# AlanConfluent/flink

Hardware: AMD Instinct MI355X
Metric: records/sec aggregated (1M-key tumbling SUM) (higher is better)
Workload: dtype int64

## Files before the change

flink_amd/_abi.py:

```python
import ctypes as C

import numpy as np

FWA_ABI_VERSION = 5
FWA_MAX_AGGS = 8
FWA_MAX_COLS = 8

TUMBLE, SLIDE, CUMULATE, SESSION = 0, 1, 2, 3
WINDOW_KINDS = {"TUMBLE": TUMBLE, "SLIDE": SLIDE, "HOP": SLIDE, "CUMULATE": CUMULATE, "SESSION": SESSION}
SEM_DATASTREAM, SEM_TABLE = 0, 1
SEMANTICS = {"DATASTREAM": SEM_DATASTREAM, "TABLE": SEM_TABLE}
KEY_JAVA_LONG, KEY_BINROW_BIGINT, KEY_PREHASHED, KEY_GROUP_PREFIXED = 0, 1, 2, 3

AGG_KINDS = {
    "COUNT": 0, "SUM_I64": 1, "SUM_F32": 2, "SUM_F64": 3, "MIN_I64": 4, "MAX_I64": 5,
    "MIN_F32": 6, "MAX_F32": 7, "MIN_F64": 8, "MAX_F64": 9, "AVG_I64": 10, "AVG_F32": 11,
    "AVG_F64": 12, "COUNT_COL": 13,
    "SUM_DEC": 14, "AVG_DEC": 15, "SUM_DEC128": 16, "AVG_DEC128": 17,
    "SUM_I32": 18, "MIN_I32": 19, "MAX_I32": 20, "FIRST_64": 21, "FIRST_32": 22,
    "MINBY_I64": 23, "MAXBY_I64": 24, "MINBY_I32": 25, "MAXBY_I32": 26, "MINBY_F64": 27, "MAXBY_F64": 28,
    "MINBY_F32": 29, "MAXBY_F32": 30, "SEL_64": 31, "SEL_32": 32,
    "COUNT_DISTINCT": 33,
}
AGG_DISTINCT = 0x100
# ... 41 lines not shown
    w = np.frombuffer(memoryview(raw).cast("B"), np.uint64).reshape(-1, 2)
    out = np.empty(w.shape[0], object)
    for i in range(w.shape[0]):
        u = int(w[i, 0]) | (int(w[i, 1]) << 64)
        out[i] = u - (1 << 128) if u >= 1 << 127 else u
    return out

STATUS = {0: "OK", -1: "E_ARG", -2: "E_TS_MIN", -3: "E_KEYGROUP", -4: "E_MERGE_LATE", -5: "E_OOM",
          -6: "E_DEVICE", -7: "E_UNSUPPORTED", -8: "E_STATE", -9: "E_CORRUPT", -10: "E_INTERNAL"}

CFG_DYNAMIC_GAP = 0x1
CFG_LATE_INDICES = 0x2
CFG_RECORD_LISTS = 0x4
CFG_REDUCE = 0x8
CFG_BY_LAST = 0x10
CFG_DISTINCT_RANGE = 0x20
CFG_DISTINCT_SESSION = 0x40
CFG_F32_FOLD = 0x80

PUSH_DEVICE_PTRS = 0x1
PUSH_ASYNC = 0x2

OPT_KEY_TABLE_SHAPE = 34
OPT_HEAP_KEY_POS = 35


def key_table_shape(value):
    return int(value) & 0xff, int(value) >> 8

LONG_MIN = -(1 << 63)
LONG_MAX = (1 << 63) - 1


class AggSpec(C.Structure):
    _fields_ = [("kind", C.c_int32), ("col", C.c_int32)]


class Config(C.Structure):
    _fields_ = [
        ("abi_version", C.c_int32), ("window_kind", C.c_int32), ("semantics", C.c_int32),
        ("key_kind", C.c_int32), ("size_ms", C.c_int64), ("slide_ms", C.c_int64),
        ("offset_ms", C.c_int64), ("gap_ms", C.c_int64), ("allowed_lateness_ms", C.c_int64),
        ("max_parallelism", C.c_int32), ("kg_start", C.c_int32), ("kg_end", C.c_int32),
        ("num_aggs", C.c_int32), ("aggs", AggSpec * FWA_MAX_AGGS), ("device", C.c_int32),
        ("output_on_device", C.c_int32), ("key_capacity", C.c_int64), ("max_batch", C.c_int64),
        ("flags", C.c_int32), ("gap_col", C.c_int32), ("tz_n", C.c_int32), ("nullable_cols", C.c_int32),
# ... 123 lines not shown
```

flink_amd/csrc/engine.hip:

```cpp
#include <hip/hip_runtime.h>
#include <hipcub/device/device_radix_sort.hpp>
#include <hipcub/device/device_scan.hpp>

#include <algorithm>
#include <cstdio>
#include <cstdlib>
#include <cstring>
#include <map>
#include <set>
#include <string>
#include <vector>

#include "../../include/flink_amd.h"
#include "java_math.h"
#include "dec_view.h"

#define LONG_MIN_J ((int64_t)0x8000000000000000LL)
#define LONG_MAX_J ((int64_t)0x7fffffffffffffffLL)

namespace {

#include "ingest.inc"
#include "ingest_launch.inc"

// ... 755 lines not shown
    int32_t slot[kRelTabN];
    uint8_t code[kRelTabN], fresh[kRelTabN];
};

__global__ void push_reset_kernel(DevStatus* st, unsigned long long* want, int32_t nwant, uint32_t* bcnt, int32_t nbcnt,
                                  int32_t* rel2slot, RelTab tab) {
    const int32_t t = blockIdx.x * blockDim.x + threadIdx.x;
    const int32_t nt = gridDim.x * blockDim.x;
    if (rel2slot) {
        uint8_t* code = (uint8_t*)(rel2slot + kRelCap);
        uint8_t* fresh = code + kRelCap;
        for (int32_t i = t; i < kRelCap; i += nt) {
            const int32_t j = i - tab.lo;
            const bool in = j >= 0 && j < tab.n;
            rel2slot[i] = in ? tab.slot[j] : -1;
            code[i] = in ? tab.code[j] : kCodeSlow;
            fresh[i] = in ? tab.fresh[j] : (uint8_t)0;
        }
    }
    if (t == 0) {
        st->error = 0; st->spill_n = 0; st->want_n = 0; st->key_full = 0;
        st->rows = 0;
        st->dropped = 0; st->late_fire = 0; st->max_q = 0; st->min_q = ~0ull; st->ovf_n = 0; st->strag_n = 0; st->wide_n = 0;
    }
    for (int32_t i = t; i < nwant; i += nt) want[i] = 0ull;
    for (int32_t i = t; i < nbcnt; i += nt) bcnt[i] = 0u;
}

struct SlotList { int32_t n, id[15]; };
__global__ void reset_slots_kernel(unsigned long long* const* slot_base, const int32_t* list, SlotList inl, int64_t stride,
                                   int32_t* touched, const EngineConst* __restrict__ cp) {
    const EngineConst& c = *cp;
    const int32_t sid = inl.n ? inl.id[blockIdx.y] : list[blockIdx.y];
    const int32_t slot = sid < 0 ? ~sid : sid;
    if (sid < 0) {
        if (blockIdx.x == 0 && threadIdx.x == 0) touched[slot] = 0;
        return;
    }
    unsigned long long* base = slot_base[slot];
    const int64_t step = (int64_t)gridDim.x * blockDim.x;
    const int64_t m = stride / 2;
    for (int col = 0; col < c.nacc; ++col) {
        const unsigned long long v = (col > 0 && c.acc_kind[col] == ACC_MIN_ORD) ? ~0ull : 0ull;
        ulonglong2* p = (ulonglong2*)(base + (int64_t)col * stride);
        const ulonglong2 v2 = make_ulonglong2(v, v);
        int64_t i = (int64_t)blockIdx.x * blockDim.x + threadIdx.x;
// ... 220 lines not shown
    bool st_ready = false;
    bool af_pend = false;
    bool af_gpu = false;
    int64_t af_rows = 0;
    int64_t* h_af_rows = nullptr;
    hipEvent_t ev_af = nullptr;
    int32_t* h_touched = nullptr;
    int32_t h_touched_cap = 0;
    bool sparse = false;
    bool red = false;
    unsigned long long* d_rk = nullptr;
    int32_t* d_iota = nullptr;
    int64_t iota_cap = 0;
    int64_t iota_n = 0;
    bool iota_pending = false, iota_ran = false;
    int32_t* d_rslots = nullptr;
    int64_t rslots_cap = 0;
    int64_t rk_cap = 0;
    int64_t red_seq_base = 0;
    SpState* sp = nullptr;
    int32_t opt_pre = -1, opt_mp = -1, opt_narrow = -1, opt_cells = -1;
    int32_t opt_variant = 0;
    int64_t stragglers = 0;
    bool rows_zero = false;
    int64_t fused_fires = 0;
    int64_t reset_launches = 0;
    int32_t push_epoch = 0;
    unsigned long long* d_rsum = nullptr;
    bool rs_valid = false;
    int64_t rs_q0 = 0;
    int32_t rs_u0 = 0, rs_epoch = 0;
    int32_t rs_k = 4;
    bool rs_on = true;
    int64_t rs_used = 0;
    int64_t opt_out_min = 0;
    bool opt_partials_v1 = false;
    int32_t opt_profile = 0;
    void* d_mf = nullptr;
    size_t mf_bytes = 0;
    double mf_groups_per_row = 1.0;
    double mf_capx = 2.0;
    int32_t opt_fire_partials = -1;
    int32_t opt_dec_wrap_null = 0;
    int32_t opt_heap_key_pos = -1;
    int64_t mf_calls = 0, mf_fallbacks = 0;
    int64_t* d_dr = nullptr;
// ... 1317 lines not shown
    int64_t qmin = LONG_MAX_J, qmax = LONG_MIN_J;
    bool republish = false;
    std::vector<int32_t> late_idx;
    for (int round = 0;; ++round) {
        if (round == 0 && status_enqueued && e->st_ready) rc = FWA_OK;
        else rc = (round == 0 && status_enqueued) ? wait_status(e) : sync_status(e);
        e->st_ready = false;
        if (rc) return rc;
        if (e->v2_timing_pending) {
            float ms = 0.f;
            HIPCHK(e, hipEventElapsedTime(&ms, e->ev[4], e->ev[5]));
            e->partition_ms += ms;
            e->ingest_ms += ms;
            HIPCHK(e, hipEventElapsedTime(&ms, e->ev[6], e->ev[7]));
            e->combine_ms += ms;
            e->ingest_ms += ms;
            e->v2_timing_pending = false;
        }
        if (!ran_v2 || round > 0) { rc = account_ingest(e); if (rc) return rc; }
        const DevStatus st = *e->h_st;
        if (ran_v2 && round == 0 && (int64_t)st.ovf_n * 64 > n) e->pre = true;
        if (ran_v2 && round == 0 && (int64_t)st.strag_n * 64 > n) e->mp = true;
        if (ran_v2 && round == 0) e->stragglers += st.strag_n;
        if (ran_v2 && round == 0 && e->narrow_used && (int64_t)st.wide_n * 64 > n) e->narrow = false;
        if (round == 0) settle_push_stale(e);
        if (st.error) {
            const char* m = st.error == FWA_E_KEYGROUP ? "Key group is not in the owned KeyGroupRange (StateTable.getMapForKeyGroup)"
                          : st.error == FWA_E_TS_MIN ? "Record has Long.MIN_VALUE timestamp (= no timestamp marker)."
                          : st.error == FWA_E_OOM ? (st.key_full ? "key table full: raise fwa_config.key_capacity" : "slice want-set overflow")
                                                  : "device error";
            return fail(e, st.error, m);
        }
        if (st.late_fire) {
            const size_t o = late_idx.size();
            late_idx.resize(o + st.late_fire);
            HIPCHK(e, hipMemcpy(late_idx.data() + o, e->d_late, 4 * (size_t)st.late_fire, hipMemcpyDeviceToHost));
        }
        dropped += (int64_t)st.dropped;
        if (st.max_q) qmax = std::max<int64_t>(qmax, jm::unord_i64(st.max_q));
        if (st.min_q != ~0ull) qmin = std::min<int64_t>(qmin, jm::unord_i64(st.min_q));
        if (round == 0) e->steady = ran_v2 && st.spill_n == 0;
        if (st.spill_n == 0) break;
        if (round > 64) return fail(e, FWA_E_STATE, "miss replay did not converge");
        std::vector<unsigned long long> want(kWantCap);
        HIPCHK(e, hipMemcpy(want.data(), e->d_want, sizeof(unsigned long long) * kWantCap, hipMemcpyDeviceToHost));
        for (unsigned long long w : want) {
// ... 1337 lines not shown
        case FWA_OPT_HEAP_KEY_POS:
            if (value < 0 || value > (e->dist ? e->dist->ucfg.num_aggs : e->dec ? e->dec->ucfg.num_aggs : e->cfg.num_aggs))
                return fail(e, FWA_E_ARG, "FWA_OPT_HEAP_KEY_POS: the key's tuple position, 0 .. num_aggs");
            e->opt_heap_key_pos = (int32_t)value;
            return FWA_OK;
        case FWA_OPT_DISTINCT_SLOTS:
            if (!e->dist) return fail(e, FWA_E_UNSUPPORTED, "FWA_OPT_DISTINCT_SLOTS: no COUNT(DISTINCT) aggregate");
            if (e->dist->d_tab) return fail(e, FWA_E_STATE, "FWA_OPT_DISTINCT_SLOTS: before the first push");
            if (value < 64 || (value & (value - 1)) || value > ((int64_t)1 << 40))
                return fail(e, FWA_E_ARG, "FWA_OPT_DISTINCT_SLOTS: a power of two >= 64");
            e->dist->first_slots = value;
            return FWA_OK;
        case FWA_OPT_F32_FOLD_SLOTS:
            if (!e->fold) return fail(e, FWA_E_UNSUPPORTED, "FWA_OPT_F32_FOLD_SLOTS: no SUM_F32 aggregate under FWA_CFG_F32_FOLD");
            if (e->fold->d_tab) return fail(e, FWA_E_STATE, "FWA_OPT_F32_FOLD_SLOTS: before the first push");
            if (value < 64 || (value & (value - 1)) || value > ((int64_t)1 << 31))
                return fail(e, FWA_E_ARG, "FWA_OPT_F32_FOLD_SLOTS: a power of two >= 64");
            e->fold->first_slots = value;
            return FWA_OK;
        case FWA_OPT_F32_FOLD_REBUILDS: case FWA_OPT_F32_FOLD_RESOLVE_US: case FWA_OPT_F32_FOLD_SORT_US:
        case FWA_OPT_F32_FOLD_RUNS_US: case FWA_OPT_F32_FOLD_ROWS_US:
        case FWA_OPT_DISTINCT_LIVE: case FWA_OPT_DISTINCT_REBUILDS: case FWA_OPT_STRAGGLERS: case FWA_OPT_KEY_TABLE_DIGEST:
        case FWA_OPT_DISTINCT_INDEX_US: case FWA_OPT_DISTINCT_COUNT_US: case FWA_OPT_DISTINCT_COUNT_STEPS:
        case FWA_OPT_FAST_SLICE_PUSHES: case FWA_OPT_KEY_TABLE_SHAPE:
            return fail(e, FWA_E_ARG, "read-only option");
        default: return fail(e, FWA_E_ARG, "unknown option");
    }
}

int fwa_get_option(const fwa_engine* e, int32_t option, int64_t* value) {
    if (!e || !value) return FWA_E_ARG;
    auto eff = [](int32_t opt, bool adaptive_on) -> int64_t { return opt == 1 || (opt != 0 && adaptive_on) ? 1 : 0; };
    switch (option) {
        case FWA_OPT_SKEW_MERGE: *value = eff(e->opt_pre, e->pre); return FWA_OK;
        case FWA_OPT_WINDOW_PASSES: *value = eff(e->opt_mp, e->mp); return FWA_OK;
        case FWA_OPT_NARROW_ENTRIES: *value = eff(e->opt_narrow, e->narrow); return FWA_OK;
        case FWA_OPT_SESSION_CELLS: *value = eff(e->opt_cells, e->cell_skip <= 0); return FWA_OK;
        case FWA_OPT_OUT_MIN_ROWS: *value = e->opt_out_min > 0 ? e->opt_out_min : ((int64_t)1 << 22); return FWA_OK;
        case FWA_OPT_PARTIALS_ONE_PASS: *value = e->opt_partials_v1 ? 1 : 0; return FWA_OK;
        case FWA_OPT_SP_TABLE: case FWA_OPT_SP_FMAX: case FWA_OPT_SP_BUDGET:
            if (!e->sp) return FWA_E_UNSUPPORTED;
            *value = option == FWA_OPT_SP_TABLE ? e->sp->T : option == FWA_OPT_SP_FMAX ? (e->sp->fmax ? e->sp->fmax : kSpMaxF)
                                                                                    : (int64_t)e->sp->budget;
            return FWA_OK;
        case FWA_OPT_PROFILE: *value = e->opt_profile; return FWA_OK;
        case FWA_OPT_SESSION_PATH: *value = e->sess_path; return FWA_OK;
        case FWA_OPT_INGEST_VARIANT: *value = e->opt_variant; return FWA_OK;
        case FWA_OPT_SLIDE_CARRIED: *value = e->rs_used; return FWA_OK;
        case FWA_OPT_FIRE_PARTIALS: *value = e->mf_calls - e->mf_fallbacks; return FWA_OK;
        case FWA_OPT_DEC_WRAP_NULL: *value = e->opt_dec_wrap_null; return FWA_OK;
        case FWA_OPT_HEAP_KEY_POS: *value = e->opt_heap_key_pos; return FWA_OK;
        case FWA_OPT_FUSED_FIRES: *value = e->fused_fires; return FWA_OK;
        case FWA_OPT_RESET_LAUNCHES: *value = e->reset_launches; return FWA_OK;
        case FWA_OPT_STALE_RETIRES: *value = e->stale_retires; return FWA_OK;
        case FWA_OPT_STRAGGLERS: *value = e->stragglers; return FWA_OK;
        case FWA_OPT_FAST_SLICE_PUSHES: *value = e->fast_slice_pushes; return FWA_OK;
        case FWA_OPT_KEY_TABLE_SHAPE:
            if (e->sparse) return FWA_E_UNSUPPORTED;
            *value = (int64_t)e->seg_log | ((int64_t)e->part_bits << 8);
            return FWA_OK;
        case FWA_OPT_KEY_TABLE_DIGEST: {
            std::vector<unsigned long long> table((size_t)e->capacity + 1);
            if (!e->d_keys || hipStreamSynchronize(e->stream) != hipSuccess ||
                hipMemcpy(table.data(), e->d_keys, 8 * table.size(), hipMemcpyDeviceToHost) != hipSuccess) return FWA_E_DEVICE;
            uint64_t h = 0xcbf29ce484222325ull;
            for (unsigned long long w : table)
                for (int b = 0; b < 8; ++b) h = (h ^ ((w >> (8 * b)) & 0xff)) * 0x100000001b3ull;
            *value = (int64_t)h;
            return FWA_OK;
        }
        case FWA_OPT_DISTINCT_SLOTS: case FWA_OPT_DISTINCT_LIVE: case FWA_OPT_DISTINCT_REBUILDS:
            if (!e->dist) return FWA_E_UNSUPPORTED;
            *value = option == FWA_OPT_DISTINCT_SLOTS ? (e->dist->slots ? e->dist->slots : e->dist->first_slots)
                   : option == FWA_OPT_DISTINCT_LIVE ? e->dist->live : e->dist->rebuilds;
            return FWA_OK;
        case FWA_OPT_F32_FOLD_SLOTS: case FWA_OPT_F32_FOLD_REBUILDS: case FWA_OPT_F32_FOLD_RESOLVE_US:
        case FWA_OPT_F32_FOLD_SORT_US: case FWA_OPT_F32_FOLD_RUNS_US: case FWA_OPT_F32_FOLD_ROWS_US:
            if (!e->fold) return FWA_E_UNSUPPORTED;
// ... 60 lines not shown
```

flink_amd/csrc/ingest.inc:

```

#ifdef FWA_KPROF
#define KPROF(p) ((p) != nullptr)
#else
#define KPROF(p) false
#endif

constexpr int kBlock = 256;
constexpr uint64_t kEmptyKey = 0x8000000000000000ull;
constexpr int kBucket = 8;
constexpr int32_t kWantCap = 1 << 14;


struct DirEntry {
    int64_t q;
    int32_t slot;
    int32_t flags;
    int64_t thr;
    int64_t first_maxts;
};

struct DevStatus {
    int32_t error;
    int32_t spill_n;
    int32_t want_n;
    int32_t key_full;
    unsigned long long dropped;
    unsigned long long n_keys;
    unsigned long long late_fire;
    unsigned long long rows;
    unsigned long long max_q;
    unsigned long long min_q;
    int32_t pad;
    int32_t pad2;
    unsigned long long sess_live;
    unsigned long long drop_n;
    int32_t ovf_n;
    int32_t strag_n;
    int32_t wide_n;
    int32_t pad3;
};

__device__ __forceinline__ void note_drop(int32_t* list, DevStatus* st, bool drop, int64_t i) {
    if (!list) return;
    const unsigned long long m = __ballot(drop);
    if (!m) return;
    const int lane = threadIdx.x & 63;
    const int ld = __ffsll((long long)m) - 1;
    unsigned long long b = 0;
    if (lane == ld) b = atomicAdd(&st->drop_n, (unsigned long long)__popcll(m));
    b = __shfl(b, ld);
    if (drop) list[b + __popcll(m & ((1ull << lane) - 1))] = (int32_t)i;
}

enum AccKind : int32_t { ACC_NONE = 0, ACC_ADD_I64 = 1, ACC_ADD_F64 = 2, ACC_MIN_ORD = 3, ACC_MAX_ORD = 4, ACC_PAYLOAD = 5 };

struct AggDesc {
    int32_t kind;
    int32_t col;
    int32_t acc;
    int32_t acc_kind;
    int32_t vslot;
    int32_t alias;
// ... 718 lines not shown
            atomicMin(&a.st->min_q, (unsigned long long)jm::ord_i64(a.q_base + (int64_t)relmin));
        }
    }
    if (relmin != ~0u)
        for (uint32_t r = relmin + (uint32_t)lane; r <= relmax; r += 64) {
            const int32_t slot = a.rel2slot[r];
            if (slot >= 0 && a.touched[slot] != a.epoch) a.touched[slot] = a.epoch;
        }
}

struct CombineArgs {
    const unsigned long long* b_key;
    const unsigned long long* b_val0;
    const unsigned long long* b_val1;
    const uint16_t* b_rel;
    const uint16_t* b_n;
    const uint32_t* b_cnt;
    int64_t capb;
    int32_t seg_log, np, sl;
    int32_t sub_major;
    const int32_t* rel2slot;
    const uint8_t* relfresh;
    int32_t stale;
    int64_t q_base;
    unsigned long long* key_table;
    unsigned long long* const* slot_base;
    int64_t stride;
    DevStatus* st;
    long long* prof;
};

__device__ __forceinline__ unsigned long long ident_of(int acc_kind) { return acc_kind == ACC_MIN_ORD ? ~0ull : 0ull; }

__device__ __forceinline__ unsigned long long carried_ord(unsigned long long raw, int kind) {
    switch (kind) {
        case FWA_MIN_I64: case FWA_MAX_I64: case FWA_MINBY_I64: case FWA_MAXBY_I64: return jm::ord_i64((int64_t)raw);
        case FWA_MIN_I32: case FWA_MAX_I32: return jm::ord_i64((int64_t)(int32_t)(uint32_t)raw);
        case FWA_MIN_F32: case FWA_MAX_F32:
            return jm::ord_bits64((uint64_t)__double_as_longlong((double)__uint_as_float((uint32_t)raw)));
        default: return jm::ord_bits64(raw);
    }
}

__device__ __forceinline__ double carried_f64(unsigned long long raw, int kind) {
    return (kind == FWA_SUM_F32 || kind == FWA_AVG_F32) ? (double)__uint_as_float((uint32_t)raw)
                                                         : __longlong_as_double((long long)raw);
// ... 67 lines not shown
            stale_range(a, s_lo_, s_hi_); \
            for (int r_ = max(s_lo_, lo + SL); r_ <= s_hi_; ++r_) if (a.relfresh[r_] == 2) ident_seg(r_); \
        } } while (0)
#define STALE_SIDE(NACC) do { \
        int s_lo_, s_hi_; \
        stale_range(a, s_lo_, s_hi_); \
        if (p == a.np - 1) stale_side<TH>(a, s_lo_, s_hi_, tid, NACC, kind_of); } while (0)

constexpr int kStragL = 256;
struct StragL {
    uint32_t g, n;
    int32_t rel, pad;
    unsigned long long x0, x1;
};

__device__ __forceinline__ uint32_t kswz(uint32_t s) { return s ^ (((s >> 5) & 3u) << 1); }


typedef __attribute__((address_space(1))) unsigned long long g_u64;
typedef const __attribute__((address_space(1))) unsigned long long* gc_u64_ptr;

constexpr int32_t kLeanEmpty = (int32_t)0x80000000;
constexpr int32_t kLeanForeign = (int32_t)0x80000001;
typedef int32_t lean_i4 __attribute__((ext_vector_type(4)));

__device__ __forceinline__ uint32_t kswz32(uint32_t s) { return s ^ (((s >> 6) & 1u) << 2); }

__device__ __forceinline__ int32_t lean_key_image(unsigned long long k) {
    if (k == kEmptyKey) return kLeanEmpty;
    const bool narrow = (int64_t)(int32_t)(uint32_t)k == (int64_t)k && (uint32_t)k - 0x80000000u > 1u;
    return narrow ? (int32_t)(uint32_t)k : kLeanForeign;
}

template <int BT>
__device__ __forceinline__ void lean_pin(const lean_i4* qa, const lean_i4* qb) {
    static_assert(BT >= 1 && BT <= 4, "batch size");
    if constexpr (BT == 1) asm volatile("" : : "v"(qa[0]), "v"(qb[0]));
    else if constexpr (BT == 2) asm volatile("" : : "v"(qa[0]), "v"(qb[0]), "v"(qa[1]), "v"(qb[1]));
    else if constexpr (BT == 3) asm volatile("" : : "v"(qa[0]), "v"(qb[0]), "v"(qa[1]), "v"(qb[1]), "v"(qa[2]), "v"(qb[2]));
    else asm volatile("" : : "v"(qa[0]), "v"(qb[0]), "v"(qa[1]), "v"(qb[1]), "v"(qa[2]), "v"(qb[2]), "v"(qa[3]), "v"(qb[3]));
}

__device__ __forceinline__ int32_t lean_match(const lean_i4& qa, const lean_i4& qb, int32_t kk) {
    int32_t t = -1;
    unsigned long long m0, m1, m2, m3, m4, m5, m6, m7;
    asm("v_cmp_eq_u32_e64 %8, %16, %17\n\t"
// ... 24 lines not shown
    const unsigned long long p = (unsigned long long)xlo * c1l;
    const uint32_t z1lo = (uint32_t)p;
    const uint32_t z1hi = (uint32_t)(p >> 32) + xlo * c1h + (s & (0u - 4u * c1l));
    const uint32_t ylo = z1lo ^ ((z1lo >> 27) | (z1hi << 5));
    const uint32_t yhi = z1hi ^ (z1hi >> 27);
    const unsigned long long q = (unsigned long long)ylo * c2l;
    const uint32_t z2lo = (uint32_t)q;
    const uint32_t z2hi = (uint32_t)(q >> 32) + __umul24(ylo, c2h) + __umul24(yhi, c2l);
    const uint32_t h = z2lo ^ ((z2lo >> 31) | (z2hi << 1));
    return h & smask & ~(uint32_t)(kBucket - 1);
}

template <bool kMax>
__device__ __forceinline__ int lean_wave_red(int v) {
    auto step = [](int x, int y) { return kMax ? max(x, y) : (int)min((uint32_t)x, (uint32_t)y); };
    v = step(v, __builtin_amdgcn_update_dpp(0, v, 0xB1, 0xf, 0xf, true));
    v = step(v, __builtin_amdgcn_update_dpp(0, v, 0x4E, 0xf, 0xf, true));
    v = step(v, __builtin_amdgcn_update_dpp(0, v, 0x141, 0xf, 0xf, true));
    v = step(v, __builtin_amdgcn_update_dpp(0, v, 0x140, 0xf, 0xf, true));
    return step(step(__builtin_amdgcn_readlane(v, 0), __builtin_amdgcn_readlane(v, 16)),
                step(__builtin_amdgcn_readlane(v, 32), __builtin_amdgcn_readlane(v, 48)));
}

template <int IT, int BT, int SL, int TH>
__device__ __forceinline__ void combine3_lean(const CombineArgs& a, const EngineConst& c) {
    extern __shared__ __attribute__((aligned(16))) unsigned char smem[];
    static_assert(IT % BT == 0, "whole batches");
    static_assert(TH / kSub == 64, "one wave per sub-bucket");
    constexpr int kWaves = TH / 64;
    const int tid = threadIdx.x, lane = tid & 63, wv = tid >> 6;
    const int p = blockIdx.x;
    const int seg = 1 << a.seg_log;
    const uint32_t smask = (uint32_t)seg - 1u;
    __shared__ StragL s_strag[kStragL];
    __shared__ int s_sn, s_first;
    int32_t* lkey = (int32_t*)smem;
    uint32_t* lcnt = (uint32_t*)(smem + (size_t)seg * 8);
    unsigned long long* lacc = (unsigned long long*)(smem + (size_t)seg * 8 + (size_t)SL * seg * 4);
    int* s_mm = (int*)(smem + (size_t)seg * 8 + (size_t)SL * seg * 4 + (size_t)SL * seg * 8);
    int* s_new = s_mm + 4 * kWaves;
    long long pt = clock64();
    long long pacc[8] = {0, 0, 0, 0, 0, 0, 0, 0};
#define PMARK(k) do { if (KPROF(a.prof)) { const long long _t = clock64(); pacc[k] += _t - pt; pt = _t; } } while (0)
    unsigned long long* gkeys = a.key_table + ((int64_t)p << a.seg_log);
    for (int i = tid; i < seg; i += TH) lkey[kswz32((uint32_t)i)] = lean_key_image(gkeys[i]);
    for (int i = tid; i < SL * seg; i += TH) { lcnt[i] = 0; lacc[i] = 0ull; }
    if (tid == 0) { *s_new = 0; s_sn = 0; s_first = 0x7fffffff; }
    if (tid < 3) { s_mm[2 * tid] = 0x7fffffff; s_mm[2 * tid + 1] = -1; }
    constexpr int64_t kChunk = (int64_t)IT * 64;
    const int my_cnt = __builtin_amdgcn_readfirstlane((int)min((int64_t)a.b_cnt[p * kSub + wv], a.capb));
    const int64_t boff = (int64_t)bucket_base(p, wv, a.np, a.sub_major) * a.capb;
    int64_t cnt = 0;
    for (int s2 = 0; s2 < kSub; ++s2) cnt = max(cnt, min((int64_t)a.b_cnt[p * kSub + s2], a.capb));
    const gc_u64_ptr bk = (const gc_u64_ptr)(a.b_key + boff);
    const __attribute__((address_space(1))) uint16_t* br = (const __attribute__((address_space(1))) uint16_t*)(a.b_rel + boff);
    int lo = 0x7fffffff;
    auto kind_of = [](int) { return (int)ACC_ADD_I64; };
    auto ident_seg = [&](int r) { stale_ident<TH>(a, r, (int64_t)p << a.seg_log, ((int64_t)p + 1) << a.seg_log, tid, 2, kind_of); };
    STALE_SIDE(2);
    auto flush = [&](int rel) {
        constexpr int kPer = 4096 / TH;
        const int w = rel & (SL - 1);
        const int32_t slot = (rel >= 0 && rel < kRelCap) ? a.rel2slot[rel] : -1;
        g_u64* base = slot >= 0 ? (g_u64*)a.slot_base[slot] : nullptr;
        const int fr = (slot >= 0 && a.relfresh) ? (int)a.relfresh[rel] : 0;
        const bool fresh = fr != 0;
        const bool all = fr == 2;
        uint32_t k[kPer];
        unsigned long long x[kPer];
        int64_t g[kPer];
#pragma unroll
// ... 78 lines not shown
            __syncthreads();
        }
        const int lo_c = lo;
        PMARK(4);
        if (KPROF(a.prof)) pacc[7] += 1;
        uint32_t miss = 0;
#pragma unroll
        for (int j0 = IT - BT; j0 >= 0; j0 -= BT) {
            lean_i4 qa[BT], qb[BT];
#pragma unroll
            for (int u = 0; u < BT; ++u) {
                qa[u] = *(const lean_i4*)&lkey[hb[j0 + u]];
                qb[u] = *(const lean_i4*)&lkey[hb[j0 + u] + 4];
            }
            lean_pin<BT>(qa, qb);
#pragma unroll
            for (int u = BT - 1; u >= 0; --u) {
                const int32_t t = lean_match(qa[u], qb[u], key[j0 + u]);
                const uint32_t b = hb[j0 + u];
                hb[j0 + u] = b + (((uint32_t)t ^ (b >> 4)) & 4u) + ((uint32_t)t & 3u);
                miss = __builtin_amdgcn_alignbit(miss, (uint32_t)t, 31);
            }
        }
        uint32_t todo = miss;
        if (!whole) {
            uint32_t ok = 0;
#pragma unroll
            for (int j = 0; j < IT; ++j) ok |= rel[j] >= 0 ? (1u << j) : 0u;
            todo &= ok;
        }
        while (todo) {
            const int jm_ = __builtin_ctz(todo);
            todo &= todo - 1u;
            int32_t kk = key[0];
            uint32_t b = hb[0];
#pragma unroll
            for (int j = 1; j < IT; ++j) { kk = jm_ == j ? key[j] : kk; b = jm_ == j ? hb[j] : b; }
            b &= ~(uint32_t)(kBucket - 1);
            int32_t found = -1;
            for (int round = 0; round <= (seg >> 2) && found < 0; ++round) {
                const uint32_t f = ((b >> 6) & 1u) << 2;
                const lean_i4 pa = *(const lean_i4*)&lkey[b + f];
                const lean_i4 pb = *(const lean_i4*)&lkey[b + (f ^ 4u)];
                const int32_t eq = lean_match(pa, pb, kk), em = lean_match(pa, pb, kLeanEmpty);
                if (eq >= 0) { found = (int32_t)(b + (uint32_t)eq); break; }
                if (em >= 0) {
                    const uint32_t sidx = b + (uint32_t)em;
                    const int32_t old = atomicCAS(&lkey[kswz32(sidx)], kLeanEmpty, kk);
                    if (old == kLeanEmpty) { found = (int32_t)sidx; atomicAdd(s_new, 1); break; }
                    if (old == kk) { found = (int32_t)sidx; break; }
                    continue;
                }
                b = (b + kBucket) & smask;
            }
// ... 19 lines not shown
                const int32_t local = (int32_t)hb[j];
                const unsigned long long x0 = (unsigned long long)(int64_t)val[j];
                if (rel[j] < lo_c) {
                    if (KPROF(a.prof)) pacc[6] += 1000000;
                    const uint32_t g = (uint32_t)(((int64_t)p << a.seg_log) + local);
                    const int si = atomicAdd(&s_sn, 1);
                    if (si < kStragL) s_strag[si] = StragL{g, 1u, rel[j], 0, x0, 0ull};
                    else strag_apply(a, c, rel[j], g, 1u, x0, 0ull);
                    continue;
                }
                const int w = rel[j] & (SL - 1);
                atomicAdd(&lcnt[w * seg + local], 1u);
                atomicAdd(&lacc[(size_t)w * seg + local], x0);
            }
        }
        PMARK(5);
    }
    __syncthreads();
    if (lo != 0x7fffffff)
        for (int r = lo; r < lo + SL; ++r) flush(r);
    STALE_ABOVE();
    __syncthreads();
    if (tid == 0 && s_sn) atomicAdd(&a.st->strag_n, s_sn);
    for (int t = tid; t < min(s_sn, kStragL); t += TH) {
        const StragL se = s_strag[t];
        strag_apply(a, c, se.rel, se.g, se.n, se.x0, se.x1);
    }
    if (*s_new) {
        for (int i = tid; i < seg; i += TH) {
            const int32_t k32 = lkey[kswz32((uint32_t)i)];
            if (k32 != kLeanEmpty && gkeys[i] == kEmptyKey) gkeys[i] = (unsigned long long)(int64_t)k32;
        }
        if (tid == 0) atomicAdd(&a.st->n_keys, (unsigned long long)*s_new);
    }
    if (KPROF(a.prof) && tid == 0) for (int q = 0; q < 8; ++q) a.prof[(int64_t)p * 8 + q] = pacc[q];
#undef PMARK
}

template <int IT, int SL, int NV, int TH, int LAYOUT, int PRE = 0, int MP = 0, int NW = 0, int LEAN = 0>
__global__ void __launch_bounds__(TH, 1) combine3_kernel(CombineArgs a, const EngineConst* __restrict__ cp) {
    if constexpr (LEAN != 0) {
        static_assert(NW == 1 && LAYOUT == 1 && NV == 1 && PRE == 0 && MP == 0, "lean body: narrow COUNT + SUM entries");
        combine3_lean<IT, LEAN, SL, TH>(a, *cp);
        return;
    }
    extern __shared__ __attribute__((aligned(16))) unsigned char smem[];
// ... 288 lines not shown
```

flink_amd/csrc/ingest_host.inc:

```

static int ensure_v2_buffers(fwa_engine* e, int64_t n, bool need_bn) {
    const int64_t per = n / ((int64_t)e->np * kSub);
    const int64_t capb = per + per / 4 + 2048;
    if (capb > e->capb) {
        for (void* p : {(void*)e->d_bkey, (void*)e->d_brel, (void*)e->d_bn, (void*)e->d_bval[0], (void*)e->d_bval[1]}) if (p) HIPCHK(e, hipFree(p));
        e->d_bkey = nullptr;
        e->d_brel = nullptr;
        e->d_bn = nullptr;
        e->d_bval[0] = e->d_bval[1] = nullptr;
        const int64_t ent = capb * e->np * kSub + 8 * kMaxPart;
        HIPCHK(e, hipMalloc(&e->d_bkey, (e->nv == 1 ? 12 : 8) * ent));
        HIPCHK(e, hipMalloc(&e->d_brel, 2 * ent));
        for (int v = 0; v < e->nv; ++v) HIPCHK(e, hipMalloc(&e->d_bval[v], 8 * ent));
        e->capb = capb;
    }
    if (need_bn && !e->d_bn) HIPCHK(e, hipMalloc(&e->d_bn, 2 * (e->capb * e->np * kSub + 8 * kMaxPart)));
    if (!e->d_bcnt) {
        HIPCHK(e, hipMalloc(&e->d_bcnt, sizeof(uint32_t) * kMaxPart * kSub));
        HIPCHK(e, hipMalloc(&e->d_rel2slot, (sizeof(int32_t) + 2) * kRelCap));
    }
    return FWA_OK;
}

static int print_phase_profile(fwa_engine* e, const char* tag, hipEvent_t a, hipEvent_t b, int nb, int nph) {
// ... 149 lines not shown
    pa.st = e->d_st;
    if (e->opt_profile && !e->d_prof) HIPCHK(e, hipMalloc(&e->d_prof, sizeof(long long) * 8 * kMaxPart));
    pa.prof = e->opt_profile ? e->d_prof : nullptr;
    return FWA_OK;
}

static void fill_combine_args(const fwa_engine* e, const V2Shape& s, const PartArgs& pa, CombineArgs& ca) {
    memset(&ca, 0, sizeof(ca));
    ca.b_key = e->d_bkey;
    ca.b_rel = e->d_brel;
    ca.b_n = s.pre ? e->d_bn : nullptr;
    ca.key_table = e->d_keys;
    ca.b_val0 = e->d_bval[0];
    ca.b_val1 = e->d_bval[1];
    ca.b_cnt = e->d_bcnt;
    ca.capb = e->capb;
    ca.seg_log = e->seg_log;
    ca.np = e->np;
    ca.sl = e->sl;
    ca.sub_major = pa.sub_major;
    ca.rel2slot = e->d_rel2slot;
    ca.relfresh = s.pre ? nullptr : (const uint8_t*)(e->d_rel2slot + kRelCap) + kRelCap;
    ca.stale = e->push_stale.empty() ? 0 : 1;
    ca.q_base = pa.q_base;
    ca.slot_base = e->d_slot_base;
    ca.stride = e->stride;
    ca.st = e->d_st;
    ca.prof = pa.prof;
}

struct P3Row { P3Key key; void (*fn)(PartArgs, const EngineConst*); };
struct C3Row { C3Key key; void (*fn)(CombineArgs, const EngineConst*); };
#define FWA_P3_ROW(NV, IT, VW, KG, PRE, W16, NW, ROLL) \
    {{NV, IT, VW, KG, PRE, W16, NW, ROLL, 0, 0}, partition3_kernel<NV, IT, 1024, VW, KG, PRE, W16, NW, ROLL>},
#define FWA_C3_ROW(IT, NV, LY, PRE, MP, NW, LEAN) \
    {{IT, NV, LY, PRE, MP, NW, LEAN}, combine3_kernel<IT, 2, NV, 1024, LY, PRE, MP, NW, LEAN>},
static const P3Row kP3Rows[] = {FWA_P3_INSTANCES(FWA_P3_ROW)};
static const C3Row kC3Rows[] = {FWA_C3_INSTANCES(FWA_C3_ROW)};
#undef FWA_P3_ROW
#undef FWA_C3_ROW

static int launch_partition3(fwa_engine* e, const V2Shape& s, const PartArgs& pa) {
    const P3Key k = p3_key(s);
    const P3Row* row = std::find_if(std::begin(kP3Rows), std::end(kP3Rows), [&](const P3Row& r) { return same_kernel(r.key, k); });
    if (row == std::end(kP3Rows)) {
        char msg[128];
// ... 52 lines not shown
```

flink_amd/engine.py:

```python
import ctypes as C
import os

import numpy as np

from . import _abi as A

_HERE = os.path.dirname(os.path.abspath(__file__))
LIB_PATH = os.path.join(_HERE, "libflink_amd.so")
_LIB = None


class EngineError(RuntimeError):
    def __init__(self, code, msg):
        super().__init__("%s: %s" % (A.STATUS.get(code, code), msg))
        self.code = code


class Blob(C.Structure):
    _fields_ = [("data", C.c_void_p), ("size", C.c_int64)]


def lib():
    global _LIB
    if _LIB is not None:
# ... 97 lines not shown


def _same_side(device, **named):
    for name, xs in named.items():
        for x in (xs if isinstance(xs, (list, tuple)) else [xs]):
            if x is not None and _is_torch_cuda(x) != device:
                raise ValueError("%s: %s columns beside %s keys" % (name, "CUDA" if not device else "host",
                                                                     "CUDA" if device else "host"))


def _check(rc, h=None, what=""):
    if rc:
        msg = lib().fwa_last_error(h).decode() if h else what
        raise EngineError(rc, msg or what)


OPTIONS = {"skew_merge": 1, "window_passes": 2, "narrow_entries": 3, "session_cells": 4, "out_min_rows": 5,
           "partials_one_pass": 6, "sp_table": 7, "sp_fmax": 8, "sp_budget": 9, "profile": 10,
           "session_path": 11, "ingest_variant": 12, "slide_carried": 13, "fire_partials": 14, "dec_wrap_null": 15,
           "fused_fires": 16, "reset_launches": 17, "distinct_slots": 18, "distinct_live": 19, "distinct_rebuilds": 20,
           "stragglers": 21, "key_table_digest": 22, "distinct_index_us": 23, "distinct_count_us": 24,
           "distinct_count_steps": 25, "stale_retires": 26, "f32_fold_slots": 27, "f32_fold_rebuilds": 28,
           "f32_fold_resolve_us": 29, "f32_fold_sort_us": 30, "f32_fold_runs_us": 31, "f32_fold_rows_us": 32,
           "fast_slice_pushes": 33, "key_table_shape": 34, "heap_key_pos": 35}
DEFAULT_OPTIONS = {}


class WindowAggregator:

    def __init__(self, cfg, options=None):
        self.cfg = cfg
        self.names = A.agg_names(cfg)
        self.h = C.c_void_p()
        self._inflight = None
        self._in_stream = None
        rc = lib().fwa_create(C.byref(cfg), C.byref(self.h))
        if rc:
            why = lib().fwa_last_error(None).decode()
            raise EngineError(rc, "fwa_create" + (": " + why if why and why != "null engine" else ""))
        for name, value in DEFAULT_OPTIONS.items():
            opt = OPTIONS[name] if name in OPTIONS else int(name)
            rc = lib().fwa_set_option(self.h, opt, int(value))
            if rc and rc != -7:
                _check(rc, self.h)
        for name, value in (options or {}).items():
            self.set_option(name, value)

# ... 364 lines not shown
```

include/flink_amd.h:

```cpp
#ifndef FLINK_AMD_H
#define FLINK_AMD_H

#include <stdint.h>

#ifdef __cplusplus
extern "C" {
#endif

#define FWA_ABI_VERSION 5
#define FWA_MAX_AGGS 8
#define FWA_MAX_COLS 8

enum fwa_window_kind { FWA_TUMBLE = 0, FWA_SLIDE = 1, FWA_CUMULATE = 2, FWA_SESSION = 3 };

enum fwa_semantics { FWA_SEM_DATASTREAM = 0, FWA_SEM_TABLE = 1 };

enum fwa_key_kind { FWA_KEY_JAVA_LONG = 0, FWA_KEY_BINROW_BIGINT = 1, FWA_KEY_PREHASHED = 2,
                    FWA_KEY_GROUP_PREFIXED = 3  };

enum fwa_agg_kind {
    FWA_COUNT = 0,
    FWA_SUM_I64 = 1,
    FWA_SUM_F32 = 2,
    FWA_SUM_F64 = 3,
// ... 212 lines not shown
    FWA_OPT_INGEST_VARIANT = 12,
    FWA_OPT_SLIDE_CARRIED = 13,
    FWA_OPT_FIRE_PARTIALS = 14,
    FWA_OPT_DEC_WRAP_NULL = 15,
    FWA_OPT_FUSED_FIRES = 16,
    FWA_OPT_RESET_LAUNCHES = 17,
    FWA_OPT_DISTINCT_SLOTS = 18,
    FWA_OPT_DISTINCT_LIVE = 19,
    FWA_OPT_DISTINCT_REBUILDS = 20,
    FWA_OPT_STRAGGLERS = 21,
    FWA_OPT_KEY_TABLE_DIGEST = 22,
    FWA_OPT_DISTINCT_INDEX_US = 23,
    FWA_OPT_DISTINCT_COUNT_US = 24,
    FWA_OPT_DISTINCT_COUNT_STEPS = 25,
    FWA_OPT_STALE_RETIRES = 26,
    FWA_OPT_F32_FOLD_SLOTS = 27,
    FWA_OPT_F32_FOLD_REBUILDS = 28,
    FWA_OPT_F32_FOLD_RESOLVE_US = 29,
    FWA_OPT_F32_FOLD_SORT_US = 30,
    FWA_OPT_F32_FOLD_RUNS_US = 31,
    FWA_OPT_F32_FOLD_ROWS_US = 32,
    FWA_OPT_FAST_SLICE_PUSHES = 33,
    FWA_OPT_KEY_TABLE_SHAPE = 34,
    FWA_OPT_HEAP_KEY_POS = 35
};
int fwa_set_option(fwa_engine* e, int32_t option, int64_t value);
int fwa_get_option(const fwa_engine* e, int32_t option, int64_t* value);

int fwa_key_groups(const int64_t* keys, const int32_t* key_hash, int64_t n, int32_t key_kind,
                   int32_t max_parallelism, int32_t parallelism, int32_t* kg_out, int32_t* op_out,
                   int32_t flags, int32_t device);

int fwa_route_rows(const int64_t* keys, const int32_t* key_hash, int64_t n, int32_t key_kind, int32_t max_parallelism,
                   int32_t parallelism, const void* const* cols, const int32_t* col_bytes, int32_t ncols, int64_t* out,
                   int64_t* counts, int32_t device, void* stream);

int fwa_unpack_rows(const int64_t* rows, int64_t n, int32_t ncols, int64_t* const* cols, int32_t device, void* stream);

enum fwa_key_field_type { FWA_KEY_FIELD_BIGINT = 0, FWA_KEY_FIELD_INT = 1, FWA_KEY_FIELD_DOUBLE = 2,
                          FWA_KEY_FIELD_STRING = 3 };
#define FWA_KEYDICT_MAX_ARITY 8
typedef struct fwa_key_strings { const int32_t* offsets; const uint8_t* bytes; } fwa_key_strings;
typedef struct fwa_key_strings_out { int32_t* offsets; uint8_t* bytes; int64_t capacity; int64_t needed; } fwa_key_strings_out;
typedef struct fwa_keydict fwa_keydict;
int fwa_keydict_create(int32_t arity, const int32_t* field_types, int32_t max_parallelism, int64_t capacity,
                       int32_t device, fwa_keydict** out);
// ... 33 lines not shown
```

Baseline: 65.18 billion.

## Add shared-memory side index for displaced keys in lean combine lookup

```diff
diff --git a/flink_amd/_abi.py b/flink_amd/_abi.py
--- a/flink_amd/_abi.py
+++ b/flink_amd/_abi.py
@@ -87,6 +87,7 @@
 PUSH_ASYNC = 0x2
 
 OPT_KEY_TABLE_SHAPE = 34
+OPT_DEFERRED_TRIPS = 36
 OPT_HEAP_KEY_POS = 35
 
 
diff --git a/flink_amd/csrc/engine.hip b/flink_amd/csrc/engine.hip
--- a/flink_amd/csrc/engine.hip
+++ b/flink_amd/csrc/engine.hip
@@ -801,6 +801,7 @@
         st->error = 0; st->spill_n = 0; st->want_n = 0; st->key_full = 0;
         st->rows = 0;
         st->dropped = 0; st->late_fire = 0; st->max_q = 0; st->min_q = ~0ull; st->ovf_n = 0; st->strag_n = 0; st->wide_n = 0;
+        st->defer_n = 0;
     }
     for (int32_t i = t; i < nwant; i += nt) want[i] = 0ull;
     for (int32_t i = t; i < nbcnt; i += nt) bcnt[i] = 0u;
@@ -1067,6 +1068,7 @@
     int32_t opt_pre = -1, opt_mp = -1, opt_narrow = -1, opt_cells = -1;
     int32_t opt_variant = 0;
     int64_t stragglers = 0;
+    int64_t deferred_trips = 0;
     bool rows_zero = false;
     int64_t fused_fires = 0;
     int64_t reset_launches = 0;
@@ -2430,6 +2432,7 @@
         if (ran_v2 && round == 0 && (int64_t)st.ovf_n * 64 > n) e->pre = true;
         if (ran_v2 && round == 0 && (int64_t)st.strag_n * 64 > n) e->mp = true;
         if (ran_v2 && round == 0) e->stragglers += st.strag_n;
+        if (ran_v2 && round == 0) e->deferred_trips += st.defer_n;
         if (ran_v2 && round == 0 && e->narrow_used && (int64_t)st.wide_n * 64 > n) e->narrow = false;
         if (round == 0) settle_push_stale(e);
         if (st.error) {
@@ -3813,7 +3816,7 @@
         case FWA_OPT_F32_FOLD_RUNS_US: case FWA_OPT_F32_FOLD_ROWS_US:
         case FWA_OPT_DISTINCT_LIVE: case FWA_OPT_DISTINCT_REBUILDS: case FWA_OPT_STRAGGLERS: case FWA_OPT_KEY_TABLE_DIGEST:
         case FWA_OPT_DISTINCT_INDEX_US: case FWA_OPT_DISTINCT_COUNT_US: case FWA_OPT_DISTINCT_COUNT_STEPS:
-        case FWA_OPT_FAST_SLICE_PUSHES: case FWA_OPT_KEY_TABLE_SHAPE:
+        case FWA_OPT_FAST_SLICE_PUSHES: case FWA_OPT_KEY_TABLE_SHAPE: case FWA_OPT_DEFERRED_TRIPS:
             return fail(e, FWA_E_ARG, "read-only option");
         default: return fail(e, FWA_E_ARG, "unknown option");
     }
@@ -3845,6 +3848,7 @@
         case FWA_OPT_RESET_LAUNCHES: *value = e->reset_launches; return FWA_OK;
         case FWA_OPT_STALE_RETIRES: *value = e->stale_retires; return FWA_OK;
         case FWA_OPT_STRAGGLERS: *value = e->stragglers; return FWA_OK;
+        case FWA_OPT_DEFERRED_TRIPS: *value = e->deferred_trips; return FWA_OK;
         case FWA_OPT_FAST_SLICE_PUSHES: *value = e->fast_slice_pushes; return FWA_OK;
         case FWA_OPT_KEY_TABLE_SHAPE:
             if (e->sparse) return FWA_E_UNSUPPORTED;
diff --git a/flink_amd/csrc/ingest.inc b/flink_amd/csrc/ingest.inc
--- a/flink_amd/csrc/ingest.inc
+++ b/flink_amd/csrc/ingest.inc
@@ -37,7 +37,7 @@
     int32_t ovf_n;
     int32_t strag_n;
     int32_t wide_n;
-    int32_t pad3;
+    int32_t defer_n;
 };
 
 __device__ __forceinline__ void note_drop(int32_t* list, DevStatus* st, bool drop, int64_t i) {
@@ -802,6 +802,7 @@
     const int32_t* rel2slot;
     const uint8_t* relfresh;
     int32_t stale;
+    int32_t side;
     int64_t q_base;
     unsigned long long* key_table;
     unsigned long long* const* slot_base;
@@ -915,6 +916,7 @@
 
 constexpr int32_t kLeanEmpty = (int32_t)0x80000000;
 constexpr int32_t kLeanForeign = (int32_t)0x80000001;
+constexpr int kSideN = 4;
 typedef int32_t lean_i4 __attribute__((ext_vector_type(4)));
 
 __device__ __forceinline__ uint32_t kswz32(uint32_t s) { return s ^ (((s >> 6) & 1u) << 2); }
@@ -985,6 +987,22 @@
                 step(__builtin_amdgcn_readlane(v, 32), __builtin_amdgcn_readlane(v, 48)));
 }
 
+__device__ __forceinline__ int32_t side_match(const lean_i4& q, int32_t kk) {
+    int32_t t = -1;
+    unsigned long long m0, m1, m2, m3;
+    asm("v_cmp_eq_u32_e64 %4, %8, %9\n\t"
+        "v_cmp_eq_u32_e64 %3, %7, %9\n\t"
+        "v_cmp_eq_u32_e64 %2, %6, %9\n\t"
+        "v_cmp_eq_u32_e64 %1, %5, %9\n\t"
+        "v_cndmask_b32_e64 %0, %0, 3, %4\n\t"
+        "v_cndmask_b32_e64 %0, %0, 2, %3\n\t"
+        "v_cndmask_b32_e64 %0, %0, 1, %2\n\t"
+        "v_cndmask_b32_e64 %0, %0, 0, %1"
+        : "+v"(t), "=&s"(m0), "=&s"(m1), "=&s"(m2), "=&s"(m3)
+        : "v"(q.x), "v"(q.y), "v"(q.z), "v"(q.w), "v"(kk));
+    return t;
+}
+
 template <int IT, int BT, int SL, int TH>
 __device__ __forceinline__ void combine3_lean(const CombineArgs& a, const EngineConst& c) {
     extern __shared__ __attribute__((aligned(16))) unsigned char smem[];
@@ -1002,14 +1020,31 @@
     unsigned long long* lacc = (unsigned long long*)(smem + (size_t)seg * 8 + (size_t)SL * seg * 4);
     int* s_mm = (int*)(smem + (size_t)seg * 8 + (size_t)SL * seg * 4 + (size_t)SL * seg * 8);
     int* s_new = s_mm + 4 * kWaves;
+    int* s_defer = s_mm + 8;
+    int32_t* lside = (int32_t*)(smem + (size_t)seg * 4);
+    uint16_t* lsslot = (uint16_t*)(smem + (size_t)seg * 6);
+    static_assert(kSideN == 4, "a side record is one 16-byte read");
     long long pt = clock64();
     long long pacc[8] = {0, 0, 0, 0, 0, 0, 0, 0};
 #define PMARK(k) do { if (KPROF(a.prof)) { const long long _t = clock64(); pacc[k] += _t - pt; pt = _t; } } while (0)
     unsigned long long* gkeys = a.key_table + ((int64_t)p << a.seg_log);
+    if (a.side)
+        for (int i = tid; i < seg / 2; i += TH) lside[i] = kLeanEmpty;
     for (int i = tid; i < seg; i += TH) lkey[kswz32((uint32_t)i)] = lean_key_image(gkeys[i]);
     for (int i = tid; i < SL * seg; i += TH) { lcnt[i] = 0; lacc[i] = 0ull; }
-    if (tid == 0) { *s_new = 0; s_sn = 0; s_first = 0x7fffffff; }
+    if (tid == 0) { *s_new = 0; *s_defer = 0; s_sn = 0; s_first = 0x7fffffff; }
     if (tid < 3) { s_mm[2 * tid] = 0x7fffffff; s_mm[2 * tid + 1] = -1; }
+    if (a.side) {
+        __syncthreads();
+        for (int i = tid; i < seg; i += TH) {
+            const int32_t k32 = lkey[kswz32((uint32_t)i)];
+            if ((uint32_t)k32 - 0x80000000u <= 1u) continue;
+            const uint32_t h = lean_home(k32, smask);
+            if (h == ((uint32_t)i & ~(uint32_t)(kBucket - 1))) continue;
+            for (int q = 0; q < kSideN; ++q)
+                if (atomicCAS(&lside[(h >> 1) + q], kLeanEmpty, k32) == kLeanEmpty) { lsslot[(h >> 1) + q] = (uint16_t)i; break; }
+        }
+    }
     constexpr int64_t kChunk = (int64_t)IT * 64;
     const int my_cnt = __builtin_amdgcn_readfirstlane((int)min((int64_t)a.b_cnt[p * kSub + wv], a.capb));
     const int64_t boff = (int64_t)bucket_base(p, wv, a.np, a.sub_major) * a.capb;
@@ -1134,6 +1169,19 @@
                 miss = __builtin_amdgcn_alignbit(miss, (uint32_t)t, 31);
             }
         }
+        if (a.side && __builtin_amdgcn_ballot_w64(miss != 0u) != 0ull) {
+#pragma unroll
+            for (int j = 0; j < IT; ++j) {
+                if (__builtin_amdgcn_ballot_w64((miss & (1u << j)) != 0u) == 0ull) continue;
+                const uint32_t r = (hb[j] & ~(uint32_t)(kBucket - 1)) >> 1;
+                const lean_i4 q = *(const lean_i4*)&lside[r];
+                const int32_t pos = side_match(q, key[j]);
+                const uint32_t sl = lsslot[r + ((uint32_t)pos & 3u)];
+                const bool hit = ((miss >> j) & 1u) != 0u && pos >= 0;
+                hb[j] = hit ? sl : hb[j];
+                miss = hit ? miss & ~(1u << j) : miss;
+            }
+        }
         uint32_t todo = miss;
         if (!whole) {
             uint32_t ok = 0;
@@ -1142,6 +1190,7 @@
             todo &= ok;
         }
         while (todo) {
+            if (__builtin_amdgcn_readfirstlane(lane) == lane) atomicAdd(s_defer, 1);
             const int jm_ = __builtin_ctz(todo);
             todo &= todo - 1u;
             int32_t kk = key[0];
@@ -1207,6 +1256,7 @@
     STALE_ABOVE();
     __syncthreads();
     if (tid == 0 && s_sn) atomicAdd(&a.st->strag_n, s_sn);
+    if (tid == 0 && *s_defer) atomicAdd(&a.st->defer_n, *s_defer);
     for (int t = tid; t < min(s_sn, kStragL); t += TH) {
         const StragL se = s_strag[t];
         strag_apply(a, c, se.rel, se.g, se.n, se.x0, se.x1);
diff --git a/flink_amd/csrc/ingest_host.inc b/flink_amd/csrc/ingest_host.inc
--- a/flink_amd/csrc/ingest_host.inc
+++ b/flink_amd/csrc/ingest_host.inc
@@ -195,6 +195,7 @@
     ca.rel2slot = e->d_rel2slot;
     ca.relfresh = s.pre ? nullptr : (const uint8_t*)(e->d_rel2slot + kRelCap) + kRelCap;
     ca.stale = e->push_stale.empty() ? 0 : 1;
+    ca.side = (e->opt_variant & 2048) ? 0 : 1;
     ca.q_base = pa.q_base;
     ca.slot_base = e->d_slot_base;
     ca.stride = e->stride;
diff --git a/flink_amd/engine.py b/flink_amd/engine.py
--- a/flink_amd/engine.py
+++ b/flink_amd/engine.py
@@ -143,7 +143,8 @@
            "stragglers": 21, "key_table_digest": 22, "distinct_index_us": 23, "distinct_count_us": 24,
            "distinct_count_steps": 25, "stale_retires": 26, "f32_fold_slots": 27, "f32_fold_rebuilds": 28,
            "f32_fold_resolve_us": 29, "f32_fold_sort_us": 30, "f32_fold_runs_us": 31, "f32_fold_rows_us": 32,
-           "fast_slice_pushes": 33, "key_table_shape": 34, "heap_key_pos": 35}
+           "fast_slice_pushes": 33, "key_table_shape": 34, "heap_key_pos": 35,
+           "deferred_trips": 36}
 DEFAULT_OPTIONS = {}
 
 
diff --git a/include/flink_amd.h b/include/flink_amd.h
--- a/include/flink_amd.h
+++ b/include/flink_amd.h
@@ -258,6 +258,7 @@
     FWA_OPT_F32_FOLD_ROWS_US = 32,
     FWA_OPT_FAST_SLICE_PUSHES = 33,
     FWA_OPT_KEY_TABLE_SHAPE = 34,
+    FWA_OPT_DEFERRED_TRIPS = 36,
     FWA_OPT_HEAP_KEY_POS = 35
 };
 int fwa_set_option(fwa_engine* e, int32_t option, int64_t value);
```

After: 64.71 billion. About the same (-0.7%).
